# eddyxzc/lpopc

Measured on AMD Instinct MI355X. Metric: eval_g+eval_jac_g calls/sec, 4-phase 4096-LGR-pt problem, higher is better.
Workload: dtype f64

## Files before the change

lpopc_amd/csrc/problems/problems.hpp:

```cpp
#pragma once
#include <type_traits>
#include <hip/hip_runtime.h>

#include "../../../include/rpm_hip.h"

namespace rpm {

#define RPM_DEV __device__ __forceinline__

template <class P, class = void> struct prob_nq { static constexpr int value = 0; };
template <class P> struct prob_nq<P, decltype(void(P::NQ))> { static constexpr int value = P::NQ; };

template <class P, class CP>
RPM_DEV void pf_dae(int ph, double t, const double* x, const double* u, const double* p, CP c, double* f, double* cp) {
  if constexpr (prob_nq<P>::value > 0) P::dae(ph, t, x, u, p, c, f, cp);
  else P::dae(ph, t, x, u, c, f, cp);
}
template <class P, class = void>
struct has_stage : std::false_type {};
template <class P>
struct has_stage<P, std::void_t<typename P::Stage>> : std::true_type {};
template <class P, class = void>
struct stage_always : std::false_type {};
template <class P>
struct stage_always<P, std::enable_if_t<P::STAGE_ALWAYS>> : std::true_type {};
template <class P, bool = has_stage<P>::value>
struct stage_of { struct type {}; };
template <class P>
struct stage_of<P, true> { using type = typename P::Stage; };

template <class P, class CP>
RPM_DEV void pf_dae_jac_col(int ph, int v, double t, const double* x, const double* u, const double* p, CP c, double* df, double* dc) {
  if constexpr (prob_nq<P>::value > 0) P::dae_jac_col(ph, v, t, x, u, p, c, df, dc);
  else P::dae_jac_col(ph, v, t, x, u, c, df, dc);
}
template <class P>
RPM_DEV double pf_lagrange(int ph, double t, const double* x, const double* u, const double* p, const double* c) {
  if constexpr (prob_nq<P>::value > 0) return P::lagrange(ph, t, x, u, p, c);
  else return P::lagrange(ph, t, x, u, c);
}
template <class P>
RPM_DEV double pf_lagrange_grad_col(int ph, int v, double t, const double* x, const double* u, const double* p, const double* c) {
  if constexpr (prob_nq<P>::value > 0) return P::lagrange_grad_col(ph, v, t, x, u, p, c);
  else return P::lagrange_grad_col(ph, v, t, x, u, c);
}
template <class P>
RPM_DEV double pf_mayer(int ph, double t0, const double* x0, double tf, const double* xf, const double* p, const double* c) {
  if constexpr (prob_nq<P>::value > 0) return P::mayer(ph, t0, x0, tf, xf, p, c);
  else return P::mayer(ph, t0, x0, tf, xf, c);
}
template <class P>
RPM_DEV double pf_mayer_grad_col(int ph, int q, double t0, const double* x0, double tf, const double* xf, const double* p, const double* c) {
  if constexpr (prob_nq<P>::value > 0) return P::mayer_grad_col(ph, q, t0, x0, tf, xf, p, c);
  else return P::mayer_grad_col(ph, q, t0, x0, tf, xf, c);
}
template <class P>
RPM_DEV void pf_event(int ph, double t0, const double* x0, double tf, const double* xf, const double* p, const double* c, double* ev) {
  if constexpr (prob_nq<P>::value > 0) P::event(ph, t0, x0, tf, xf, p, c, ev);
  else P::event(ph, t0, x0, tf, xf, c, ev);
}
template <class P>
RPM_DEV void pf_event_jac_col(int ph, int v, double t0, const double* x0, double tf, const double* xf, const double* p, const double* c, double* de) {
  if constexpr (prob_nq<P>::value > 0) P::event_jac_col(ph, v, t0, x0, tf, xf, p, c, de);
  else P::event_jac_col(ph, v, t0, x0, tf, xf, c, de);
}
template <class P>
RPM_DEV void pf_link(int lph, int rph, const double* xl, const double* xr, const double* pl, const double* pr, const double* c, int nlink, double* lo) {
  if constexpr (prob_nq<P>::value > 0) P::link(lph, rph, xl, xr, pl, pr, c, nlink, lo);
  else P::link(lph, rph, xl, xr, c, nlink, lo);
}
template <class P>
RPM_DEV void pf_link_jac_col(int lph, int rph, int v, const double* xl, const double* xr, const double* pl, const double* pr, const double* c, int nlink, double* dl) {
  if constexpr (prob_nq<P>::value > 0) P::link_jac_col(lph, rph, v, xl, xr, pl, pr, c, nlink, dl);
  else P::link_jac_col(lph, rph, v, xl, xr, c, nlink, dl);
}

RPM_DEV double cube_rn(double x) {
  const double p = x * x, ep = fma(x, x, -p);
  const double q = p * x, eq = fma(p, x, -q);
  return q + (eq + ep * x);
}

struct LaunchProblem {
  static constexpr int ID = RPM_PROBLEM_LAUNCH;
  static constexpr int NX = 7, NU = 3, NC = 1, NE_MAX = 5, NLINK_MAX = 7, NCONST = 22;
  static constexpr bool HAS_ANALYTIC = false;

  template <class CP = const double*>
  RPM_DEV static void dae(int ph, double t, const double* x, const double* u, CP c,
                          double* f, double* p) {
    (void)t;
    const double r0 = x[0], r1 = x[1], r2 = x[2], m = x[6];
    const double rad = sqrt((r0 * r0 + r1 * r1) + r2 * r2);
    double vrel[3];
#pragma unroll
    for (int cc = 0; cc < 3; ++cc) {
      double ocr = 0.0;
      ocr += r0 * c[cc + 0];
      ocr += r1 * c[cc + 3];
      ocr += r2 * c[cc + 6];
      vrel[cc] = x[3 + cc] - ocr;
    }
    const double speedrel = sqrt((vrel[0] * vrel[0] + vrel[1] * vrel[1]) + vrel[2] * vrel[2]);
    const double altitude = rad - c[14];
    const double rho = exp(-altitude / c[13]) * c[12];
    const double bc = rho / (m * 2) * (c[11] * c[10]);
    const double bcspeed = bc * speedrel;
    const double mu3 = (1.0 * c[9]) / cube_rn(rad);
    double T_tot, mdot;
    if (ph == 1 || ph == 2) {
      const double T_srb = 1.0 * ((ph == 1 ? 6 : 3) * c[16]);
      const double T_first = 1.0 * c[17];
      T_tot = T_srb + T_first;
      double m1dot = 0.0, m2dot = 0.0;
      m1dot -= T_srb / (c[15] * c[19]);
      m2dot -= T_first / (c[15] * c[20]);
      mdot = m1dot + m2dot;
    } else if (ph == 3) {
      T_tot = 1.0 * c[17];
      mdot = 0.0;
      mdot -= T_tot / (c[15] * c[20]);
    } else {
      T_tot = 1.0 * c[18];
      mdot = 0.0;
      mdot -= T_tot / (c[15] * c[21]);
    }
    p[0] = (u[0] * u[0] + u[1] * u[1]) + u[2] * u[2];
    const double Toverm = T_tot / m;
#pragma unroll
    for (int j = 0; j < 3; ++j) {
      const double drag = (bcspeed * (-1.0)) * vrel[j];
      const double grav = (-mu3) * x[j];
      f[j] = x[3 + j];
      f[3 + j] = (Toverm * u[j] + drag) + grav;
    }
    f[6] = mdot;
  }

  struct Stage { double ocr[3], vrel[3], rho, mu3, speedrel, bc, T_tot, mdot; };
// ... 93 lines not shown
                            const double* c, double* ev) {
    (void)t0; (void)x0; (void)tf;
    if (ph != 4) return;
    const double mu = c[9];
    const double* rv = xf;
    const double* vv = xf + 3;
    double hv[3], nv[3], e3[3];
    hv[0] = rv[1] * vv[2] - rv[2] * vv[1];
    hv[1] = rv[2] * vv[0] - rv[0] * vv[2];
    hv[2] = rv[0] * vv[1] - rv[1] * vv[0];
    nv[0] = 0.0 * hv[2] - 1.0 * hv[1];
    nv[1] = 1.0 * hv[0] - 0.0 * hv[2];
    nv[2] = 0.0 * hv[1] - 0.0 * hv[0];
    const double n = sqrt(dot3(nv, nv));
    const double h2 = dot3(hv, hv);
    const double v2 = dot3(vv, vv);
    const double r = sqrt(dot3(rv, rv));
    const double s1 = v2 - mu / r, s2 = dot3(rv, vv);
#pragma unroll
    for (int j = 0; j < 3; ++j) e3[j] = (rv[j] * s1 - vv[j] * s2) * (1.0 / mu);
    const double p = h2 / mu;
    const double e = sqrt(dot3(e3, e3));
    const double twopi = 2 * 3.14159265358979323846;
    double Om1 = acos(nv[0] / n);
    if (nv[1] < 0 - 2.220446049250313e-16) Om1 = twopi - Om1;
    double Om2 = acos(dot3(nv, e3) / n / e);
    if (e3[2] < 0) Om2 = twopi - Om2;
    ev[0] = p / (1 - e * e);
    ev[1] = e;
    ev[2] = acos(hv[2] / sqrt(h2));
    ev[3] = Om1;
    ev[4] = Om2;
  }
  RPM_DEV static void link(int lph, int rph, const double* xfl, const double* x0r, const double* c,
                           int nlink, double* out) {
    (void)lph; (void)rph; (void)c;
    for (int j = 0; j < nlink; ++j) out[j] = x0r[j] - xfl[j];
  }
  RPM_DEV static double mayer(int ph, double t0, const double* x0, double tf, const double* xf,
                              const double* c) {
    (void)t0; (void)x0; (void)tf; (void)c;
    return ph == 4 ? -xf[6] : 0.0;
  }
  RPM_DEV static double lagrange(int ph, double t, const double* x, const double* u, const double* c) {
    (void)ph; (void)t; (void)x; (void)u; (void)c;
    return 0.0;
  }
};

struct HypersensitiveProblem {
  static constexpr int ID = RPM_PROBLEM_HYPERSENSITIVE;
  static constexpr int NX = 1, NU = 1, NC = 0, NE_MAX = 0, NLINK_MAX = 0, NCONST = 0;
  static constexpr bool HAS_ANALYTIC = true;
  template <class CP = const double*>
  RPM_DEV static void dae(int, double, const double* x, const double* u, CP, double* f, double*) {
    f[0] = ((-x[0]) * x[0]) * x[0] + u[0];
  }
  template <class CP = const double*>
  RPM_DEV static void dae_jac_col(int, int v, double, const double* x, const double*, CP,
                                  double* df, double*) {
    df[0] = (v == 0) ? -3 * (x[0] * x[0]) : (v == 1 ? 1.0 : 0.0);
  }
  RPM_DEV static void event(int, double, const double*, double, const double*, const double*, double*) {}
  RPM_DEV static void link(int, int, const double*, const double*, const double*, int, double*) {}
  RPM_DEV static double mayer(int, double, const double*, double, const double*, const double*) { return 0.0; }
  RPM_DEV static double lagrange(int, double, const double* x, const double* u, const double*) {
    return 0.5 * (x[0] * x[0] + u[0] * u[0]);
  }
  RPM_DEV static double lagrange_grad_col(int, int v, double, const double* x, const double* u, const double*) {
    return v == 0 ? x[0] : (v == 1 ? u[0] : 0.0);
  }
  RPM_DEV static double mayer_grad_col(int, int, double, const double*, double, const double*, const double*) {
    return 0.0;
  }
  RPM_DEV static void event_jac_col(int, int, double, const double*, double, const double*, const double*, double*) {}
  RPM_DEV static void link_jac_col(int, int, int, const double*, const double*, const double*, int, double*) {}
};

struct BrysonDenhamProblem {
  static constexpr int ID = RPM_PROBLEM_BRYSON_DENHAM;
  static constexpr int NX = 3, NU = 1, NC = 0, NE_MAX = 5, NLINK_MAX = 0, NCONST = 0;
  static constexpr bool HAS_ANALYTIC = false;
  template <class CP = const double*>
  RPM_DEV static void dae(int, double, const double* x, const double* u, CP, double* f, double*) {
    f[0] = x[1];
    f[1] = u[0];
    f[2] = 0.5 * (u[0] * u[0]);
  }
  RPM_DEV static void event(int, double, const double* x0, double, const double* xf, const double*, double* ev) {
    ev[0] = x0[0]; ev[1] = x0[1]; ev[2] = x0[2]; ev[3] = xf[0]; ev[4] = xf[1];
  }
  RPM_DEV static void link(int, int, const double*, const double*, const double*, int, double*) {}
  RPM_DEV static double mayer(int, double, const double*, double, const double* xf, const double*) { return xf[2]; }
  RPM_DEV static double lagrange(int, double, const double*, const double*, const double*) { return 0.0; }
};

struct BrachistochroneProblem {
  static constexpr int ID = RPM_PROBLEM_BRACHISTOCHRONE;
  static constexpr int NX = 3, NU = 1, NC = 0, NE_MAX = 5, NLINK_MAX = 0, NCONST = 1;
  static constexpr bool HAS_ANALYTIC = true;
  template <class CP = const double*>
  RPM_DEV static void dae(int, double, const double* x, const double* u, CP c, double* f, double*) {
    const double sn = sin(u[0]), cs = cos(u[0]);
    f[0] = x[2] * sn;
    f[1] = x[2] * cs;
    f[2] = c[0] * cs;
  }
  template <class CP = const double*>
  RPM_DEV static void dae_jac_col(int, int v, double, const double* x, const double* u, CP c,
                                  double* df, double*) {
    const double sn = sin(u[0]), cs = cos(u[0]);
    df[0] = df[1] = df[2] = 0.0;
    if (v == 2) { df[0] = sn; df[1] = cs; }
    if (v == 3) { df[0] = x[2] * cs; df[1] = -(x[2] * sn); df[2] = -(c[0] * sn); }
  }
  RPM_DEV static void event(int, double, const double* x0, double, const double* xf, const double*, double* ev) {
    ev[0] = x0[0]; ev[1] = x0[1]; ev[2] = x0[2]; ev[3] = xf[0]; ev[4] = xf[1];
  }
  RPM_DEV static void event_jac_col(int, int v, double, const double*, double, const double*, const double*, double* de) {
    for (int i = 0; i < 5; ++i) de[i] = 0.0;
    if (v < 3) de[v] = 1.0;
    if (v == 4) de[3] = 1.0;
    if (v == 5) de[4] = 1.0;
  }
  RPM_DEV static void link(int, int, const double*, const double*, const double*, int, double*) {}
  RPM_DEV static void link_jac_col(int, int, int, const double*, const double*, const double*, int, double*) {}
  RPM_DEV static double mayer(int, double, const double*, double tf, const double*, const double*) { return tf; }
  RPM_DEV static double mayer_grad_col(int, int v, double, const double*, double, const double*, const double*) {
    return v == 2 * NX + 1 ? 1.0 : 0.0;
  }
  RPM_DEV static double lagrange(int, double, const double*, const double*, const double*) { return 0.0; }
  RPM_DEV static double lagrange_grad_col(int, int, double, const double*, const double*, const double*) { return 0.0; }
};

struct MinTimeClimbProblem {
  static constexpr int ID = RPM_PROBLEM_MIN_TIME_CLIMB;
  static constexpr int NX = 4, NU = 1, NC = 0, NE_MAX = 7, NLINK_MAX = 0, NCONST = 10;
  static constexpr bool HAS_ANALYTIC = false;
  template <class CP = const double*>
  RPM_DEV static void dae(int, double, const double* x, const double* u, CP c, double* f, double*) {
    const double h = x[0], v = x[1], gam = x[2], m = x[3], al = u[0];
    const double r = h + c[0];
    const double rho = c[5] * exp(-h / c[6]);
    const double as = c[7] - c[8] * h;
    const double M = v / as;
    const double ch = cosh((M - 1.0) / 0.06);
    const double CLa = 3.44 + 1.0 / (ch * ch);
    const double CD0 = 0.013 + 0.0144 * (1.0 + tanh((M - 0.98) / 0.06));
    const double eta = 0.54 + 0.15 * (1.0 + tanh((M - 0.9) / 0.06));
    const double CD = CD0 + eta * CLa * (al * al);
    const double CL = CLa * al;
    const double q = 0.5 * rho * v * v;
    const double D = q * c[2] * CD;
    const double Lf = q * c[2] * CL;
    const double T = c[9] * pow(rho / c[5], 0.7) * (1.0 + 0.3 * M);
    const double sg = sin(gam), cg = cos(gam), sa = sin(al), ca = cos(al);
    f[0] = v * sg;
    f[1] = (T * ca - D) / m - c[1] * sg / (r * r);
    f[2] = (T * sa + Lf) / (m * v) + cg * (v / r - c[1] / (v * (r * r)));
    f[3] = -T / (c[3] * c[4]);
  }
  RPM_DEV static void event(int, double, const double* x0, double, const double* xf, const double*, double* ev) {
    ev[0] = x0[0]; ev[1] = x0[1]; ev[2] = x0[2]; ev[3] = x0[3]; ev[4] = xf[0]; ev[5] = xf[1]; ev[6] = xf[2];
  }
  RPM_DEV static void link(int, int, const double*, const double*, const double*, int, double*) {}
  RPM_DEV static double mayer(int, double, const double*, double tf, const double*, const double*) { return tf; }
  RPM_DEV static double lagrange(int, double, const double*, const double*, const double*) { return 0.0; }
};

struct QuadrotorProblem {
  static constexpr int ID = RPM_PROBLEM_QUADROTOR;
  static constexpr int NX = 12, NU = 4, NC = 0, NE_MAX = 0, NLINK_MAX = 0, NCONST = 15;
  static constexpr bool HAS_ANALYTIC = false;
  template <class CP = const double*>
  RPM_DEV static void dae(int, double, const double* x, const double* f4, CP c, double* f, double*) {
    const double ph = x[6], th = x[7], ps = x[8], p = x[9], q = x[10], r = x[11];
    const double F = ((f4[0] + f4[1]) + f4[2]) + f4[3];
    const double tx = c[2] * (f4[1] - f4[3]);
    const double ty = c[2] * (f4[2] - f4[0]);
    const double tz = c[6] * (((f4[0] - f4[1]) + f4[2]) - f4[3]);
    double sph, cph, sth, cth, sps, cps;
    sincos(ph, &sph, &cph);
    sincos(th, &sth, &cth);
    sincos(ps, &sps, &cps);
    const double b3x = cph * sth * cps + sph * sps;
    const double b3y = cph * sth * sps - sph * cps;
    const double b3z = cph * cth;
    const double Fm = F / c[0];
    f[0] = x[3];
    f[1] = x[4];
    f[2] = x[5];
    f[3] = Fm * b3x;
    f[4] = Fm * b3y;
    f[5] = Fm * b3z - c[1];
    const double w = q * sph + r * cph;
    f[6] = p + w * (sth / cth);
    f[7] = q * cph - r * sph;
    f[8] = w / cth;
    f[9] = (tx - (c[5] - c[4]) * q * r) / c[3];
    f[10] = (ty - (c[3] - c[5]) * p * r) / c[4];
    f[11] = (tz - (c[4] - c[3]) * p * q) / c[5];
  }
  struct Stage { double sph, cph, sth, cth, sps, cps; };
  static constexpr bool STAGE_ALWAYS = true;
  template <class CP = const double*>
  RPM_DEV static void stage(int, double, const double* x, const double*, CP, Stage& s) {
    sincos(x[6], &s.sph, &s.cph);
    sincos(x[7], &s.sth, &s.cth);
    sincos(x[8], &s.sps, &s.cps);
  }
  template <class CP = const double*>
  RPM_DEV static void dae_from(int, double, const double* x, const double* f4, CP c, const Stage& base, int var, double* f, double*) {
    Stage s = base;
    if (var == 6) sincos(x[6], &s.sph, &s.cph);
    else if (var == 7) sincos(x[7], &s.sth, &s.cth);
    else if (var == 8) sincos(x[8], &s.sps, &s.cps);
    const double p = x[9], q = x[10], r = x[11];
    const double F = ((f4[0] + f4[1]) + f4[2]) + f4[3];
    const double tx = c[2] * (f4[1] - f4[3]);
    const double ty = c[2] * (f4[2] - f4[0]);
    const double tz = c[6] * (((f4[0] - f4[1]) + f4[2]) - f4[3]);
    const double sph = s.sph, cph = s.cph, sth = s.sth, cth = s.cth, sps = s.sps, cps = s.cps;
    const double b3x = cph * sth * cps + sph * sps;
    const double b3y = cph * sth * sps - sph * cps;
    const double b3z = cph * cth;
    const double Fm = F / c[0];
    f[0] = x[3];
    f[1] = x[4];
    f[2] = x[5];
    f[3] = Fm * b3x;
    f[4] = Fm * b3y;
    f[5] = Fm * b3z - c[1];
    const double w = q * sph + r * cph;
    f[6] = p + w * (sth / cth);
    f[7] = q * cph - r * sph;
    f[8] = w / cth;
    f[9] = (tx - (c[5] - c[4]) * q * r) / c[3];
    f[10] = (ty - (c[3] - c[5]) * p * r) / c[4];
    f[11] = (tz - (c[4] - c[3]) * p * q) / c[5];
  }
  template <class CP = const double*>
  RPM_DEV static void dae_from2(int ph, double t, const double* x, const double* f4, CP c, const Stage& base, int va, int vb, double* f, double* p) {
    Stage s = base;
    if (va == 6 || vb == 6) sincos(x[6], &s.sph, &s.cph);
    if (va == 7 || vb == 7) sincos(x[7], &s.sth, &s.cth);
    if (va == 8 || vb == 8) sincos(x[8], &s.sps, &s.cps);
    dae_from(ph, t, x, f4, c, s, -1, f, p);
  }
  RPM_DEV static void event(int, double, const double*, double, const double*, const double*, double*) {}
  RPM_DEV static void link(int, int, const double*, const double*, const double*, int, double*) {}
  RPM_DEV static double mayer(int, double, const double*, double, const double*, const double*) { return 0.0; }
  RPM_DEV static double lagrange(int, double, const double* x, const double* f4, const double* c) {
    const double hov = c[0] * c[1] / 4.0;
    const double d0 = x[0] - c[7], d1 = x[1] - c[8], d2 = x[2] - c[9];
    const double ep = (d0 * d0 + d1 * d1) + d2 * d2;
    const double evv = (x[3] * x[3] + x[4] * x[4]) + x[5] * x[5];
    const double ea = (x[6] * x[6] + x[7] * x[7]) + x[8] * x[8];
    const double ew = (x[9] * x[9] + x[10] * x[10]) + x[11] * x[11];
    const double u0 = f4[0] - hov, u1 = f4[1] - hov, u2 = f4[2] - hov, u3 = f4[3] - hov;
    const double eu = ((u0 * u0 + u1 * u1) + u2 * u2) + u3 * u3;
    return (((c[10] * ep + c[11] * evv) + c[12] * ea) + c[13] * ew) + c[14] * eu;
  }
};

struct ParamSledProblem {
  static constexpr int ID = RPM_PROBLEM_PARAM_SLED;
  static constexpr int NX = 2, NU = 1, NQ = 1, NC = 0, NE_MAX = 4, NLINK_MAX = 0, NCONST = 1;
  static constexpr bool HAS_ANALYTIC = true;
  template <class CP = const double*>
  RPM_DEV static void dae(int, double, const double* x, const double* u, const double* p, CP, double* f, double*) {
    f[0] = x[1];
    f[1] = p[0] * u[0];
  }
  RPM_DEV static void event(int, double, const double* x0, double, const double* xf, const double*, const double*, double* ev) {
    ev[0] = x0[0];
    ev[1] = x0[1];
    ev[2] = xf[0];
    ev[3] = xf[1];
  }
  RPM_DEV static void link(int, int, const double*, const double*, const double*, const double*, const double*, int, double*) {}
  RPM_DEV static double mayer(int, double, const double*, double tf, const double*, const double* p, const double* c) {
    return tf + c[0] * (p[0] * p[0]);
  }
  RPM_DEV static double lagrange(int, double, const double*, const double*, const double*, const double*) { return 0.0; }
  template <class CP = const double*>
  RPM_DEV static void dae_jac_col(int, int v, double, const double*, const double* u, const double* p, CP, double* df, double*) {
    df[0] = (v == 1) ? 1.0 : 0.0;
    df[1] = (v == 2) ? p[0] : (v == 4 ? u[0] : 0.0);
  }
  RPM_DEV static void event_jac_col(int, int v, double, const double*, double, const double*, const double*, const double*, double* de) {
    de[0] = (v == 0) ? 1.0 : 0.0;
    de[1] = (v == 1) ? 1.0 : 0.0;
    de[2] = (v == 3) ? 1.0 : 0.0;
    de[3] = (v == 4) ? 1.0 : 0.0;
  }
  RPM_DEV static void link_jac_col(int, int, int, const double*, const double*, const double*, const double*, const double*, int, double*) {}
  RPM_DEV static double mayer_grad_col(int, int q, double, const double*, double, const double*, const double* p, const double* c) {
    return q == 5 ? 1.0 : (q == 6 ? 2.0 * c[0] * p[0] : 0.0);
  }
  RPM_DEV static double lagrange_grad_col(int, int, double, const double*, const double*, const double*, const double*) { return 0.0; }
};

struct ParamOscProblem {
  static constexpr int ID = RPM_PROBLEM_PARAM_OSC;
  static constexpr int NX = 2, NU = 1, NQ = 2, NC = 1, NE_MAX = 2, NLINK_MAX = 4, NCONST = 2;
  static constexpr bool HAS_ANALYTIC = false;
  template <class CP = const double*>
  RPM_DEV static void dae(int, double, const double* x, const double* u, const double* p, CP c, double* f, double* cp) {
    f[0] = x[1];
    f[1] = (-(p[0] * x[0]) - c[0] * x[1]) + u[0];
    cp[0] = x[0] + p[1] * u[0];
  }
  RPM_DEV static void event(int ph, double, const double* x0, double, const double* xf, const double* p, const double*, double* ev) {
    if (ph == 1) {
      ev[0] = x0[0];
      ev[1] = x0[1];
    } else {
      ev[0] = xf[0] + p[1];
    }
  }
  RPM_DEV static void link(int, int, const double* xl, const double* xr, const double* pl, const double* pr, const double*, int, double* lo) {
    lo[0] = xl[0] - xr[0];
    lo[1] = xl[1] - xr[1];
    lo[2] = pl[0] - pr[0];
    lo[3] = pl[1] - pr[1];
  }
  RPM_DEV static double mayer(int ph, double, const double*, double, const double* xf, const double* p, const double*) {
    return ph == 2 ? xf[0] * xf[0] + p[0] * p[1] : 0.0;
  }
  RPM_DEV static double lagrange(int, double, const double* x, const double* u, const double* p, const double* c) {
    return (u[0] * u[0] + p[1] * (x[0] * x[0])) + c[1] * (p[0] * p[0]);
  }
};

}
```

lpopc_amd/csrc/rpm_tile_kernels.hip:

```cpp
#include "rpm_device_internal.hpp"

namespace rpm {


template <class Prob, bool WG, bool WJ, bool AN, bool WAVE = false>
__device__ void endpoint_block(const KParams& K, const TaskDev task, const double* __restrict__ x,
                               double* __restrict__ g, double* __restrict__ vals, double* lds, int inst) {
  constexpr int NX = Prob::NX, NQ = prob_nq<Prob>::value, NQs = NQ > 0 ? NQ : 1;
  bool bad_g = false, bad_j = false;
  constexpr int NE = Prob::NE_MAX > 0 ? Prob::NE_MAX : 1;
  constexpr int NL = Prob::NLINK_MAX > 0 ? Prob::NLINK_MAX : 1;
  static_assert(!WAVE || 2 * NX + 3 + 2 * NQ <= 64, "endpoint perturbations must fit one wave");
  const int tid = WAVE ? int(threadIdx.x & 63) : int(threadIdx.x);
  const int nthr = WAVE ? 64 : int(blockDim.x);
  const double* c = K.consts + size_t(inst) * K.consts_stride;
  if (task.type == 0) {
    for (int r = tid; r < K.P + K.L; r += nthr) {
      if (WG) {
        double acc = 0.0;
        acc += K.alin_v[2 * r] * x[K.alin_j[2 * r]];
        acc += K.alin_v[2 * r + 1] * x[K.alin_j[2 * r + 1]];
        g[K.m_nl + r] = acc;
        chk_note(bad_g, acc);
      }
      if (WJ) {
        vals[K.nnz_nl + 2 * r] = K.alin_v[2 * r];
        vals[K.nnz_nl + 2 * r + 1] = K.alin_v[2 * r + 1];
      }
    }
  } else if (task.type == 1) {
    const PhaseDev ph = K.phases[task.idx];
    const int pi = tid;
    const bool act = pi <= 2 * NX + 2 + NQ;
    double x0[NX], xf[NX], ev[NE], pp[NQs];
#pragma unroll
    for (int j = 0; j < NQ; ++j) pp[j] = x[ph.x_t0 + 2 + j];
    double t0 = x[ph.x_t0], tf = x[ph.x_t0 + 1];
#pragma unroll
    for (int j = 0; j < NX; ++j) {
      x0[j] = x[ph.x_state0 + j * (ph.N + 1)];
      xf[j] = x[ph.x_state0 + j * (ph.N + 1) + ph.N];
    }
    double h = 1.0;
    if (WJ && !AN && pi >= 1) {
      const int v = pi - 1;
#pragma unroll
      for (int j = 0; j < NX; ++j) {
        if (v == j) { h = K.tol * (fabs(x0[j]) + 1); x0[j] += h; }
        if (v == NX + 1 + j) { h = K.tol * (fabs(xf[j]) + 1); xf[j] += h; }
      }
      if (v == NX) { h = K.tol * (1 + fabs(t0)); t0 += h; }
      if (v == 2 * NX + 1) { h = K.tol * (1 + fabs(tf)); tf += h; }
#pragma unroll
// ... 71 lines not shown
      }
    }
#pragma unroll
    for (int i = 0; i < NL; ++i) lo[i] = 0.0;
    if (act && (pi == 0 || !AN)) pf_link<Prob>(lk.left + 1, lk.right + 1, xl, xr, ql, qr, c, lk.nlink, lo);
    double base[NL];
    if constexpr (WAVE) {
#pragma unroll
      for (int i = 0; i < NL; ++i) base[i] = __shfl(lo[i], 0, 64);
    }
    if (pi == 0) {
#pragma unroll
      for (int i = 0; i < NL; ++i)
        if (i < lk.nlink) {
          if (!WAVE) lds[i] = lo[i];
          if (WG) { g[lk.g0 + i] = lo[i]; chk_note(bad_g, lo[i]); }
        }
    }
    if constexpr (!WAVE) {
      __syncthreads();
#pragma unroll
      for (int i = 0; i < NL; ++i) base[i] = lds[i];
    }
    if (WJ && act && pi >= 1) {
      const int v = pi - 1;
      double dl[NL];
      if constexpr (AN) {
        pf_link_jac_col<Prob>(lk.left + 1, lk.right + 1, v, xl, xr, ql, qr, c, lk.nlink, dl);
      } else {
#pragma unroll
        for (int i = 0; i < NL; ++i) dl[i] = (lo[i] - base[i]) / (1.0 * h);
      }
#pragma unroll
      for (int i = 0; i < NL; ++i)
        if (i < lk.nlink) { vals[lk.v0 + v * lk.nlink + i] = dl[i]; chk_note(bad_j, dl[i]); }
    }
  }
  chk_report(K.chk, bad_g, bad_j);
}


template <class Prob, bool WJ, bool AN, bool STG = false, class CP>
__device__ __forceinline__ void role_dynamics(int phase_num, int role, double tk, const double* xs, const double* us, CP c,
                                              double* f, double* cp,
                                              const typename stage_of<Prob>::type* base_stage = nullptr) {
  const int v = role - 1;
  if constexpr (STG) {
    Prob::dae_from(phase_num, tk, xs, us, c, *base_stage, (WJ && role >= 1) ? v : -1, f, cp);
  } else if (!AN || role == 0) {
    pf_dae<Prob>(phase_num, tk, xs, us, us + Prob::NU, c, f, cp);
  } else if constexpr (AN) {
    pf_dae_jac_col<Prob>(phase_num, v, tk, xs, us, us + Prob::NU, c, f, cp);
  }
}

template <int NX, int NU, int NQ>
__device__ __forceinline__ double perturb_uniform(int v, double pv, double tol, double* xs, double* us, double& tk) {
  const double h = tol * (1 + fabs(pv));
  const double pp = pv + h;
#pragma unroll
  for (int i = 0; i < NX; ++i) xs[i] = (v == i) ? pp : xs[i];
#pragma unroll
  for (int j = 0; j < NU; ++j) us[j] = (v == NX + j) ? pp : us[j];
  tk = (v == NX + NU) ? pp : tk;
#pragma unroll
  for (int j = 0; j < NQ; ++j) us[NU + j] = (v == NX + NU + 1 + j) ? pp : us[NU + j];
  return h;
}

template <class Prob, int T, bool WG, bool CHK>
__device__ __forceinline__ void publish_base(const double* f, const double* cp, double* Fb, int kk, double* g, int g0, int N,
                                             int k, bool& bad_g) {
  constexpr int NX = Prob::NX, NC = Prob::NC;
#pragma unroll
  for (int i = 0; i < NX; ++i) Fb[i * T + kk] = f[i];
#pragma unroll
  for (int j = 0; j < NC; ++j) {
    Fb[(NX + j) * T + kk] = cp[j];
    if (WG) {
      g[g0 + (NX + j) * N + k] = cp[j];
      if (CHK) chk_note(bad_g, cp[j]);
    }
  }
}

template <int T, bool CHK>
__device__ __forceinline__ void store_defect(int sv, double dx, double tspan, const double* Fb, int kk, double* g, int g0,
                                             int N, int k, bool& bad_g) {
  const double dfc = dx - Fb[sv * T + kk] * (tspan / 2.0);
  g[g0 + sv * N + k] = dfc;
  if (CHK) chk_note(bad_g, dfc);
}

__device__ __forceinline__ int xcd_place(int b, int count) {
  const int per = count >> 3, rem = count & 7, xcd = b & 7;
  return xcd * per + (xcd < rem ? xcd : rem) + (b >> 3);
}

#define RPM_REC(rec, f) __builtin_amdgcn_readfirstlane((rec)[offsetof(TileDev, f) / 4])

template <class Prob, int T, bool WG, bool WJ, bool AN, bool DXM = false>
__global__ void rpm_tile_kernel(const KParams K, const double* __restrict__ xall,
                                double* __restrict__ gall, double* __restrict__ vall) {
  constexpr int NX = Prob::NX, NU = Prob::NU, NC = Prob::NC, NQ = prob_nq<Prob>::value;
  constexpr int NO = NX + NC;
  constexpr int NV = NX + NU + 1 + NQ;
// ... 60 lines not shown
  const int sv = WJ ? role - 1 : role;
  double dx = 0.0;
  if (WG && !DXM && sv >= 0 && sv < NX) {
    const double* drow = Ds + (nd.drow_off - tl.drow0);
    const double* xcol = Xs + sv * K.max_span + (nd.dcol0 - tl.span0);
    for (int j = 0; j < nd.dlen; ++j) dx += drow[j] * xcol[j];
  }
  if constexpr (DXM && WG) {
    if (tid < 64) {
      typedef double d4 __attribute__((ext_vector_type(4)));
      const int lr = tid & 15, kq = tid >> 4;
      const int ksteps = (tl.span_len + 3) >> 2;
      for (int rb = 0; rb < T; rb += 16) {
        const int row = rb + lr;
        const bool row_ok = row < tl.cnt;
        const NodeDev ndr = K.nodes[ph.node0 + tl.k0 + (row_ok ? row : tl.cnt - 1)];
        const int rel0 = ndr.dcol0 - tl.span0;
        const double* drow = Ds + (ndr.drow_off - tl.drow0);
        for (int cb = 0; cb < NX; cb += 16) {
          const int st = cb + lr;
          d4 acc = {0.0, 0.0, 0.0, 0.0};
          for (int s = 0; s < ksteps; ++s) {
            const int kcol = 4 * s + kq;
            const int rel = kcol - rel0;
            const double a = (row_ok && rel >= 0 && rel < ndr.dlen) ? drow[rel] : 0.0;
            const double b = (st < NX && kcol < tl.span_len) ? Xs[st * K.max_span + kcol] : 0.0;
            acc = __builtin_amdgcn_mfma_f64_16x16x4f64(a, b, acc, 0, 0, 0);
          }
#pragma unroll
          for (int i = 0; i < 4; ++i) {
            const int orow = rb + kq + 4 * i;
            if (st < NX && orow < tl.cnt) DXs[st * T + orow] = acc[i];
          }
        }
      }
    }
  }

  double h = 1.0;
  const int v = role - 1;
  if (WJ && !AN && role >= 1) {
#pragma unroll
    for (int i = 0; i < NX; ++i)
      if (v == i) { h = K.tol * (1 + fabs(xs[i])); xs[i] += h; }
#pragma unroll
    for (int j = 0; j < NU; ++j)
      if (v == NX + j) { h = K.tol * (1 + fabs(us[j])); us[j] += h; }
    if (v == NX + NU) { h = K.tol * (1 + fabs(tk)); tk += h; }
#pragma unroll
    for (int j = 0; j < NQ; ++j)
      if (v == NX + NU + 1 + j) { h = K.tol * (1 + fabs(us[NU + j])); us[NU + j] += h; }
  }
  double f[NX > 0 ? NX : 1], cp[NCs];
  role_dynamics<Prob, WJ, AN>(ph.phase_num, role, tk, xs, us, c, f, cp);
  if (role == 0 && act) publish_base<Prob, T, WG, true>(f, cp, Fb, kk, g, ph.g0, ph.N, k, bad_g);
  __syncthreads();

  if (act) {
    const int N = ph.N;
    if (WG && sv >= 0 && sv < NX) store_defect<T, true>(sv, DXM ? DXs[sv * T + kk] : dx, tspan, Fb, kk, g, ph.g0, N, k, bad_g);
    if (WJ && role >= 1) {
      double J[NO];
#pragma unroll
      for (int o = 0; o < NO; ++o) {
        const double pert = o < NX ? f[o < NX ? o : 0] : cp[o >= NX ? o - NX : 0];
        J[o] = AN ? pert : (pert - Fb[o * T + kk]) / h;
      }
      double* vb = vals + ph.v_nl0 + k;
      if (v != NX + NU) {
        const int bv = v < NX + NU ? v : v + 1;
#pragma unroll
        for (int o = 0; o < NO; ++o) {
          double val;
          if (o < NX) {
            const double ret = J[o] * (tf - t0) / 2.0;
            val = (o == v) ? ddiag - ret : -ret;
          } else {
            val = J[o];
          }
          vb[size_t(o * NB + bv) * N] = val;
          chk_note(bad_j, val);
        }
      } else {
        const double a0 = -(tau * 0.5) + 0.5, af = (tau * 0.5) + 0.5;
#pragma unroll
        for (int o = 0; o < NO; ++o) {
          double v0, vf;
          if (o < NX) {
            const double fb = Fb[o * T + kk];
            const double dt = J[o] * (tf - t0) / 2.0;
            v0 = fb * (0.5) - a0 * dt;
            vf = -fb * (0.5) + af * dt;
          } else {
            v0 = a0 * J[o];
            vf = af * J[o];
          }
          vb[size_t(o * NB + NX + NU) * N] = v0;
          vb[size_t(o * NB + NX + NU + 1) * N] = vf;
          chk_note(bad_j, v0);
          chk_note(bad_j, vf);
        }
      }
    }
  }
  chk_report(K.chk, bad_g, bad_j);

  if (WJ && !K.skip_const) {
    const double* __restrict__ src = K.doff_vals + tl.c_src0;
    double* __restrict__ dst = vals + tl.c_dst0;
#pragma unroll
    for (int u = 0; u < CPRE; ++u) {
      const int q = tid + u * nthr;
      if (q < tl.c_cnt) {
#pragma unroll
        for (int i = 0; i < NX; ++i) dst[size_t(i) * tl.c_stride + q] = cpre[u];
      }
    }
    for (int q = tid + CPRE * nthr; q < tl.c_cnt; q += nthr) {
      const double dv = src[q];
// ... 38 lines not shown
  const int k = tl.k0 + kc;
  const int nidx = ph.node0 + k;
  const double tau = K.points[nidx];
  const NodeDev nd = K.nodes[nidx];
  const double ddiag = WJ ? K.diag[nidx] : 0.0;
  for (int q = tid; q < NX * tl.span_len; q += NTHR) {
    const int i = q / tl.span_len, r = q - i * tl.span_len;
    Xs[i * K.max_span + r] = x[ph.x_state0 + i * (ph.N + 1) + tl.span0 + r];
  }
  for (int q = tid; q < NU * tl.cnt; q += NTHR) {
    const int j = q / tl.cnt, r = q - j * tl.cnt;
    Us[j * T + r] = x[ph.x_control0 + j * ph.N + tl.k0 + r];
  }
  if (WG)
    for (int q = tid; q < tl.drow_len; q += NTHR) Ds[q] = K.dvals[tl.drow0 + q];
  const double t0 = x[ph.x_t0], tf = x[ph.x_t0 + 1];
  RPM_TRC(1);
  __syncthreads();
  RPM_TRC(2);

  const bool node_ok = kk < tl.cnt;
  const double tspan = tf - t0;
  const double tk0 = (tau + 1) * (tspan / 2.0) + t0;
  const int N = ph.N;
  bool first = true, no_chk = false;
  for (int role = grp; role < R || first; role += RG) {
    const bool act = node_ok && role < R;
    double xs[NX > 0 ? NX : 1], us[NU + NQ > 0 ? NU + NQ : 1];
#pragma unroll
    for (int i = 0; i < NX; ++i) xs[i] = Xs[i * K.max_span + (k - tl.span0)];
#pragma unroll
    for (int j = 0; j < NU; ++j) us[j] = Us[j * T + kc];
#pragma unroll
    for (int j = 0; j < NQ; ++j) us[NU + j] = x[ph.x_t0 + 2 + j];
    double tk = tk0;
    const int sv = WJ ? role - 1 : role;
    double dx = 0.0;
    if (WG && sv >= 0 && sv < NX) {
      const double* drow = Ds + (nd.drow_off - tl.drow0);
      const double* xcol = Xs + sv * K.max_span + (nd.dcol0 - tl.span0);
      for (int j = 0; j < nd.dlen; ++j) dx += drow[j] * xcol[j];
    }
    double h = 1.0;
    const int v = role - 1;
    if (WJ && !AN && role >= 1) {
      double pv;
      if (v < NX) pv = Xs[v * K.max_span + (k - tl.span0)];
      else if (v < NX + NU) pv = Us[(v - NX) * T + kc];
      else if (v == NX + NU) pv = tk;
      else pv = x[ph.x_t0 + 1 + (v - NX - NU)];
      h = perturb_uniform<NX, NU, NQ>(v, pv, K.tol, xs, us, tk);
    }
    double f[NX > 0 ? NX : 1], cp[NCs];
    role_dynamics<Prob, WJ, AN>(ph.phase_num, role, tk, xs, us, c, f, cp);
    if (first) {
      if (role == 0 && act) publish_base<Prob, T, WG, false>(f, cp, Fb, kk, g, ph.g0, N, k, no_chk);
      __syncthreads();
      RPM_TRC(3);
      first = false;
    }
    if (act) {
      if (WG && sv >= 0 && sv < NX) store_defect<T, false>(sv, dx, tspan, Fb, kk, g, ph.g0, N, k, no_chk);
      if (WJ && role >= 1) {
        double J[NO];
#pragma unroll
        for (int o = 0; o < NO; ++o) {
          const double pert = o < NX ? f[o < NX ? o : 0] : cp[o >= NX ? o - NX : 0];
          J[o] = AN ? pert : (pert - Fb[o * T + kk]) / h;
        }
        double* vb = vals + ph.v_nl0 + k;
        if (v != NX + NU) {
          const int bv = v < NX + NU ? v : v + 1;
#pragma unroll
          for (int o = 0; o < NO; ++o) {
            double val;
            if (o < NX) {
              const double ret = J[o] * (tf - t0) / 2.0;
              val = (o == v) ? ddiag - ret : -ret;
            } else {
              val = J[o];
            }
            vb[size_t(o * NB + bv) * N] = val;
          }
        } else {
          const double a0 = -(tau * 0.5) + 0.5, af = (tau * 0.5) + 0.5;
#pragma unroll
          for (int o = 0; o < NO; ++o) {
            double v0, vf;
            if (o < NX) {
              const double fb = Fb[o * T + kk];
              const double dt = J[o] * (tf - t0) / 2.0;
              v0 = fb * (0.5) - a0 * dt;
              vf = -fb * (0.5) + af * dt;
            } else {
              v0 = a0 * J[o];
              vf = af * J[o];
            }
            vb[size_t(o * NB + NX + NU) * N] = v0;
            vb[size_t(o * NB + NX + NU + 1) * N] = vf;
          }
        }
      }
    }
  }
  RPM_TRC(4);
  if (WJ && !K.skip_const) {
    const double* __restrict__ src = K.doff_vals + tl.c_src0;
    double* __restrict__ dst = vals + tl.c_dst0;
    const int lead = int((reinterpret_cast<size_t>(dst) >> 3) & 15);
    for (int q = tid - lead; q < tl.c_cnt; q += NTHR) {
      if (q >= 0) {
        const double dv = src[q];
#pragma unroll
        for (int i = 0; i < NX; ++i) dst[size_t(i) * tl.c_stride + q] = dv;
      }
    }
  }
#ifdef RPM_DIAG
  RPM_TRC(5);
  if (K.trace) {
    __builtin_amdgcn_s_waitcnt(0);
// ... 293 lines not shown
      for (int j = 0; j < NU; ++j) us0[j] = Us[j * T + kc];
      const double tau0 = cur[S_TAU + kc], t00 = cur[S_TT], tf0 = cur[S_TT + 1];
      Prob::stage(phase_num, (tau0 + 1) * ((tf0 - t00) / 2.0) + t00, xs0, us0, c4, base_stage);
    }
    for (int role = grp; role < R || first; role += RG) {
      const bool act = node_ok && role < R;
#ifdef RPM_DIAG
      const bool trc = role == 5;
      if (trc) { RPM_PTRC(jt, 24); }
#endif
      double xs[NXs], us[NUs];
#pragma unroll
      for (int i = 0; i < NX; ++i) xs[i] = Xs[i * K.max_span + (k - span0)];
#pragma unroll
      for (int j = 0; j < NU; ++j) us[j] = Us[j * T + kc];
#pragma unroll
      for (int j = 0; j < NQ; ++j) us[NU + j] = cur[S_TT + 2 + j];
      double tk;
      {
        const double tau = cur[S_TAU + kc], t0 = cur[S_TT], tf = cur[S_TT + 1];
        tk = (tau + 1) * ((tf - t0) / 2.0) + t0;
      }
      const int sv = WJ ? role - 1 : role;
      double dx = 0.0;
      if (WG && !DXM && sv >= 0 && sv < NX) {
        const NodeDev nd = reinterpret_cast<const NodeDev*>(cur + S_ND)[kc];
        const double* drow = Ds + (nd.drow_off - drow0);
        const double* xcol = Xs + sv * K.max_span + (nd.dcol0 - span0);
        int j = 0;
        for (; j + 4 <= nd.dlen; j += 4) {
          const double d0 = drow[j], d1 = drow[j + 1], d2 = drow[j + 2], d3 = drow[j + 3];
          const double x0 = xcol[j], x1 = xcol[j + 1], x2 = xcol[j + 2], x3 = xcol[j + 3];
          dx += d0 * x0;
          dx += d1 * x1;
          dx += d2 * x2;
          dx += d3 * x3;
        }
        for (; j < nd.dlen; ++j) dx += drow[j] * xcol[j];
      }
#ifdef RPM_DIAG
      if (trc) { if (dx == 1e300) xs[0] = 0; RPM_PTRC(jt, 25); }
#endif
      double h = 1.0;
      const int v = role - 1;
      if (WJ && !AN && role >= 1) {
        double pv;
        if (v < NX) pv = Xs[v * K.max_span + (k - span0)];
        else if (v < NX + NU) pv = Us[(v - NX) * T + kc];
        else if (v == NX + NU) pv = tk;
        else pv = cur[S_TT + 1 + (v - NX - NU)];
        h = perturb_uniform<NX, NU, NQ>(v, pv, K.tol, xs, us, tk);
      }
      double f[NXs], cp[NCs];
      role_dynamics<Prob, WJ, AN, STG>(phase_num, role, tk, xs, us, c4, f, cp, &base_stage);
#ifdef RPM_DIAG
      if (trc) { if (f[0] == 1e300) cp[0] = 0; RPM_PTRC(jt, 26); }
#endif
      if (first) {
        if (role == 0 && act) publish_base<Prob, T, WG, false>(f, cp, Fb, kk, g, g0, N, k, no_chk);
        if (grp < 4) { RPM_PTRC(jt, grp * 4 + 1); }
        if (grp == 0) {
          __hip_atomic_store(fb_ready, jt + 1, __ATOMIC_RELEASE, __HIP_MEMORY_SCOPE_WORKGROUP);
        } else {
          while (__hip_atomic_load(fb_ready, __ATOMIC_ACQUIRE, __HIP_MEMORY_SCOPE_WORKGROUP) < jt + 1)
            __builtin_amdgcn_s_sleep(1);
        }
        if (grp < 4) { RPM_PTRC(jt, grp * 4 + 2); }
        first = false;
      }
      if (act) {
        const double tau = cur[S_TAU + kc], t0 = cur[S_TT], tf = cur[S_TT + 1];
        const double ddiag = cur[S_DG + kc];
        if (WG && sv >= 0 && sv < NX) {
          if constexpr (DXM) {
            while (__hip_atomic_load(dx_ready, __ATOMIC_ACQUIRE, __HIP_MEMORY_SCOPE_WORKGROUP) < NDMA * (jt + 1)) __builtin_amdgcn_s_sleep(1);
            dx = DXs[sv * T + kk];
          }
          store_defect<T, false>(sv, dx, tf - t0, Fb, kk, g, g0, N, k, no_chk);
        }
        if (WJ && role >= 1) {
          double J[NO];
#pragma unroll
          for (int o = 0; o < NO; ++o) {
            const double pert = o < NX ? f[o < NX ? o : 0] : cp[o >= NX ? o - NX : 0];
            J[o] = AN ? pert : (pert - Fb[o * T + kk]) / h;
          }
          double* __restrict__ vb = vals + v_nl0;
          if (v != NX + NU) {
            const int bv = v < NX + NU ? v : v + 1;
#pragma unroll
            for (int o = 0; o < NO; ++o) {
              double val;
              if (o < NX) {
                const double ret = J[o] * (tf - t0) / 2.0;
                val = (o == v) ? ddiag - ret : -ret;
              } else {
                val = J[o];
              }
              (vb + size_t(o * NB + bv) * N)[k] = val;
            }
          } else {
            const double a0 = -(tau * 0.5) + 0.5, af = (tau * 0.5) + 0.5;
#pragma unroll
            for (int o = 0; o < NO; ++o) {
              double v0, vf;
              if (o < NX) {
                const double fb = Fb[o * T + kk];
                const double dt = J[o] * (tf - t0) / 2.0;
                v0 = fb * (0.5) - a0 * dt;
                vf = -fb * (0.5) + af * dt;
              } else {
                v0 = a0 * J[o];
                vf = af * J[o];
              }
              (vb + size_t(o * NB + NX + NU) * N)[k] = v0;
              (vb + size_t(o * NB + NX + NU + 1) * N)[k] = vf;
            }
          }
        }
      }
#ifdef RPM_DIAG
      if (trc) { RPM_PTRC(jt, 27); }
#endif
    }
    if (grp < 4) { RPM_PTRC(jt, grp * 4 + 3); }
    if (jt == n_iter - 1) { RPM_PEDGE_MAX(23); }
  }
}

static size_t pl_lds_bytes(int nx, int nu, int nc, int nq, const KParams& kp, bool dxm) {
  const PlLds L(nx, nu, nc, nq, kp.max_span, kp.max_drow, kp.max_cshare, true, dxm);
  return size_t(pl_shape(nx + nu + 2 + nq).NH) * L.half * sizeof(double);
}

void tile_pipeline_setup(Engine& e, Device* d, const ProblemDims& pd, int device_id) {
    int ncu = 0;
    if (hipDeviceGetAttribute(&ncu, hipDeviceAttributeMultiprocessorCount, device_id) != hipSuccess || ncu <= 0) ncu = 256;
    const int max_c = d->kp.max_cshare;
// ... 153 lines not shown
```

Before: 651,300.

## Skip time-perturbation dynamics for autonomous problems and use reciprocal FD division

Adds an AUTONOMOUS trait to every problem. For those problems the finite-difference role that perturbs time (role 1+NX+NU) reuses the base dynamics from shared memory instead of re-evaluating the DAE, since f does not depend on t. It also replaces the per-output division by h with one reciprocal plus an FMA-corrected quotient, and falls back to true division when operands are outside a safe exponent range. This removes one dynamics evaluation per column and several f64 divides, at the cost of extra branching and range checks.

Result: no change. 653,100 (median of 4 runs) (+0.3%).

```diff
diff --git a/lpopc_amd/csrc/problems/problems.hpp b/lpopc_amd/csrc/problems/problems.hpp
--- a/lpopc_amd/csrc/problems/problems.hpp
+++ b/lpopc_amd/csrc/problems/problems.hpp
@@ -21,6 +21,10 @@
 template <class P>
 struct has_stage<P, std::void_t<typename P::Stage>> : std::true_type {};
 template <class P, class = void>
+struct prob_autonomous : std::false_type {};
+template <class P>
+struct prob_autonomous<P, std::enable_if_t<P::AUTONOMOUS>> : std::true_type {};
+template <class P, class = void>
 struct stage_always : std::false_type {};
 template <class P>
 struct stage_always<P, std::enable_if_t<P::STAGE_ALWAYS>> : std::true_type {};
@@ -85,6 +89,7 @@
   static constexpr int ID = RPM_PROBLEM_LAUNCH;
   static constexpr int NX = 7, NU = 3, NC = 1, NE_MAX = 5, NLINK_MAX = 7, NCONST = 22;
   static constexpr bool HAS_ANALYTIC = false;
+  static constexpr bool AUTONOMOUS = true;
 
   template <class CP = const double*>
   RPM_DEV static void dae(int ph, double t, const double* x, const double* u, CP c,
@@ -284,6 +289,7 @@
   static constexpr int ID = RPM_PROBLEM_HYPERSENSITIVE;
   static constexpr int NX = 1, NU = 1, NC = 0, NE_MAX = 0, NLINK_MAX = 0, NCONST = 0;
   static constexpr bool HAS_ANALYTIC = true;
+  static constexpr bool AUTONOMOUS = true;
   template <class CP = const double*>
   RPM_DEV static void dae(int, double, const double* x, const double* u, CP, double* f, double*) {
     f[0] = ((-x[0]) * x[0]) * x[0] + u[0];
@@ -313,6 +319,7 @@
   static constexpr int ID = RPM_PROBLEM_BRYSON_DENHAM;
   static constexpr int NX = 3, NU = 1, NC = 0, NE_MAX = 5, NLINK_MAX = 0, NCONST = 0;
   static constexpr bool HAS_ANALYTIC = false;
+  static constexpr bool AUTONOMOUS = true;
   template <class CP = const double*>
   RPM_DEV static void dae(int, double, const double* x, const double* u, CP, double* f, double*) {
     f[0] = x[1];
@@ -331,6 +338,7 @@
   static constexpr int ID = RPM_PROBLEM_BRACHISTOCHRONE;
   static constexpr int NX = 3, NU = 1, NC = 0, NE_MAX = 5, NLINK_MAX = 0, NCONST = 1;
   static constexpr bool HAS_ANALYTIC = true;
+  static constexpr bool AUTONOMOUS = true;
   template <class CP = const double*>
   RPM_DEV static void dae(int, double, const double* x, const double* u, CP c, double* f, double*) {
     const double sn = sin(u[0]), cs = cos(u[0]);
@@ -369,6 +377,7 @@
   static constexpr int ID = RPM_PROBLEM_MIN_TIME_CLIMB;
   static constexpr int NX = 4, NU = 1, NC = 0, NE_MAX = 7, NLINK_MAX = 0, NCONST = 10;
   static constexpr bool HAS_ANALYTIC = false;
+  static constexpr bool AUTONOMOUS = true;
   template <class CP = const double*>
   RPM_DEV static void dae(int, double, const double* x, const double* u, CP c, double* f, double*) {
     const double h = x[0], v = x[1], gam = x[2], m = x[3], al = u[0];
@@ -404,6 +413,7 @@
   static constexpr int ID = RPM_PROBLEM_QUADROTOR;
   static constexpr int NX = 12, NU = 4, NC = 0, NE_MAX = 0, NLINK_MAX = 0, NCONST = 15;
   static constexpr bool HAS_ANALYTIC = false;
+  static constexpr bool AUTONOMOUS = true;
   template <class CP = const double*>
   RPM_DEV static void dae(int, double, const double* x, const double* f4, CP c, double* f, double*) {
     const double ph = x[6], th = x[7], ps = x[8], p = x[9], q = x[10], r = x[11];
@@ -499,6 +509,7 @@
   static constexpr int ID = RPM_PROBLEM_PARAM_SLED;
   static constexpr int NX = 2, NU = 1, NQ = 1, NC = 0, NE_MAX = 4, NLINK_MAX = 0, NCONST = 1;
   static constexpr bool HAS_ANALYTIC = true;
+  static constexpr bool AUTONOMOUS = true;
   template <class CP = const double*>
   RPM_DEV static void dae(int, double, const double* x, const double* u, const double* p, CP, double* f, double*) {
     f[0] = x[1];
@@ -537,6 +548,7 @@
   static constexpr int ID = RPM_PROBLEM_PARAM_OSC;
   static constexpr int NX = 2, NU = 1, NQ = 2, NC = 1, NE_MAX = 2, NLINK_MAX = 4, NCONST = 2;
   static constexpr bool HAS_ANALYTIC = false;
+  static constexpr bool AUTONOMOUS = true;
   template <class CP = const double*>
   RPM_DEV static void dae(int, double, const double* x, const double* u, const double* p, CP c, double* f, double* cp) {
     f[0] = x[1];
diff --git a/lpopc_amd/csrc/rpm_fd_div.hpp b/lpopc_amd/csrc/rpm_fd_div.hpp
--- /dev/null
+++ b/lpopc_amd/csrc/rpm_fd_div.hpp
@@ -0,0 +1,58 @@
+#pragma once
+
+#if defined(__HIP__) || defined(__CUDACC__)
+#define RPM_FD_HD __host__ __device__ inline __attribute__((always_inline))
+#else
+#define RPM_FD_HD inline
+#endif
+
+namespace rpm {
+
+constexpr double FD_SAFE_LO = 0x1p-500, FD_SAFE_HI = 0x1p+500;
+
+struct FdRecip { double h, r; bool ok; };
+
+RPM_FD_HD FdRecip fd_recip(double h) {
+  const double ah = __builtin_fabs(h);
+  return FdRecip{h, 1.0 / h, ah >= FD_SAFE_LO && ah <= FD_SAFE_HI};
+}
+
+RPM_FD_HD double fd_quot_step(const FdRecip& rc, double a, bool& safe) {
+  const double q0 = a * rc.r;
+  const double e = __builtin_fma(-rc.h, q0, a);
+  const double aa = __builtin_fabs(a);
+  unsigned long long bits;
+  __builtin_memcpy(&bits, &a, sizeof bits);
+  safe = bool(int(safe) & ((int(aa >= FD_SAFE_LO) & int(aa <= FD_SAFE_HI)) | int(bits == 0)));
+  return __builtin_fma(e, rc.r, q0);
+}
+
+RPM_FD_HD double fd_quot(const FdRecip& rc, double a) {
+  bool safe = rc.ok;
+  const double q = fd_quot_step(rc, a, safe);
+  return safe ? q : a / rc.h;
+}
+
+template <int N, class Num>
+RPM_FD_HD void fd_quot_column(const FdRecip& rc, Num num, double* q) {
+  constexpr int G = 4;
+#if defined(__clang__)
+#pragma unroll
+#endif
+  for (int o0 = 0; o0 < N; o0 += G) {
+    double a[G];
+    bool safe = rc.ok;
+#if defined(__clang__)
+#pragma unroll
+#endif
+    for (int o = o0; o < (o0 + G < N ? o0 + G : N); ++o) q[o] = fd_quot_step(rc, a[o - o0] = num(o), safe);
+    if (!safe) {
+#if defined(__clang__)
+#pragma unroll
+#endif
+      for (int o = o0; o < (o0 + G < N ? o0 + G : N); ++o) q[o] = a[o - o0] / rc.h;
+    }
+  }
+}
+
+}
diff --git a/lpopc_amd/csrc/rpm_tile_kernels.hip b/lpopc_amd/csrc/rpm_tile_kernels.hip
--- a/lpopc_amd/csrc/rpm_tile_kernels.hip
+++ b/lpopc_amd/csrc/rpm_tile_kernels.hip
@@ -1,4 +1,5 @@
 #include "rpm_device_internal.hpp"
+#include "rpm_fd_div.hpp"
 
 namespace rpm {
 
@@ -176,6 +177,18 @@
   } else if constexpr (AN) {
     pf_dae_jac_col<Prob>(phase_num, v, tk, xs, us, us + Prob::NU, c, f, cp);
   }
+}
+
+template <class Prob, bool WJ, bool AN>
+__device__ __forceinline__ bool role_repeats_base(int role) {
+  return prob_autonomous<Prob>::value && WJ && !AN && role == 1 + Prob::NX + Prob::NU;
+}
+template <class Prob, int T>
+__device__ __forceinline__ void fetch_base(const double* Fb, int kk, double* f, double* cp) {
+#pragma unroll
+  for (int i = 0; i < Prob::NX; ++i) f[i] = Fb[i * T + kk];
+#pragma unroll
+  for (int j = 0; j < Prob::NC; ++j) cp[j] = Fb[(Prob::NX + j) * T + kk];
 }
 
 template <int NX, int NU, int NQ>
@@ -342,19 +355,23 @@
       if (v == NX + NU + 1 + j) { h = K.tol * (1 + fabs(us[NU + j])); us[NU + j] += h; }
   }
   double f[NX > 0 ? NX : 1], cp[NCs];
-  role_dynamics<Prob, WJ, AN>(ph.phase_num, role, tk, xs, us, c, f, cp);
+  const bool repeats = role_repeats_base<Prob, WJ, AN>(role);
+  if (!repeats) role_dynamics<Prob, WJ, AN>(ph.phase_num, role, tk, xs, us, c, f, cp);
   if (role == 0 && act) publish_base<Prob, T, WG, true>(f, cp, Fb, kk, g, ph.g0, ph.N, k, bad_g);
   __syncthreads();
+  if (repeats) fetch_base<Prob, T>(Fb, kk, f, cp);
 
   if (act) {
     const int N = ph.N;
     if (WG && sv >= 0 && sv < NX) store_defect<T, true>(sv, DXM ? DXs[sv * T + kk] : dx, tspan, Fb, kk, g, ph.g0, N, k, bad_g);
     if (WJ && role >= 1) {
       double J[NO];
-#pragma unroll
-      for (int o = 0; o < NO; ++o) {
-        const double pert = o < NX ? f[o < NX ? o : 0] : cp[o >= NX ? o - NX : 0];
-        J[o] = AN ? pert : (pert - Fb[o * T + kk]) / h;
+      const auto pert = [&](int o) { return o < NX ? f[o < NX ? o : 0] : cp[o >= NX ? o - NX : 0]; };
+      if constexpr (AN) {
+#pragma unroll
+        for (int o = 0; o < NO; ++o) J[o] = pert(o);
+      } else {
+        fd_quot_column<NO>(fd_recip(h), [&](int o) { return pert(o) - Fb[o * T + kk]; }, J);
       }
       double* vb = vals + ph.v_nl0 + k;
       if (v != NX + NU) {
@@ -499,7 +516,8 @@
       h = perturb_uniform<NX, NU, NQ>(v, pv, K.tol, xs, us, tk);
     }
     double f[NX > 0 ? NX : 1], cp[NCs];
-    role_dynamics<Prob, WJ, AN>(ph.phase_num, role, tk, xs, us, c, f, cp);
+    if (role_repeats_base<Prob, WJ, AN>(role) && !first) fetch_base<Prob, T>(Fb, kk, f, cp);
+    else role_dynamics<Prob, WJ, AN>(ph.phase_num, role, tk, xs, us, c, f, cp);
     if (first) {
       if (role == 0 && act) publish_base<Prob, T, WG, false>(f, cp, Fb, kk, g, ph.g0, N, k, no_chk);
       __syncthreads();
@@ -510,10 +528,12 @@
       if (WG && sv >= 0 && sv < NX) store_defect<T, false>(sv, dx, tspan, Fb, kk, g, ph.g0, N, k, no_chk);
       if (WJ && role >= 1) {
         double J[NO];
-#pragma unroll
-        for (int o = 0; o < NO; ++o) {
-          const double pert = o < NX ? f[o < NX ? o : 0] : cp[o >= NX ? o - NX : 0];
-          J[o] = AN ? pert : (pert - Fb[o * T + kk]) / h;
+        const auto pert = [&](int o) { return o < NX ? f[o < NX ? o : 0] : cp[o >= NX ? o - NX : 0]; };
+        if constexpr (AN) {
+#pragma unroll
+          for (int o = 0; o < NO; ++o) J[o] = pert(o);
+        } else {
+          fd_quot_column<NO>(fd_recip(h), [&](int o) { return pert(o) - Fb[o * T + kk]; }, J);
         }
         double* vb = vals + ph.v_nl0 + k;
         if (v != NX + NU) {
@@ -913,7 +933,8 @@
         h = perturb_uniform<NX, NU, NQ>(v, pv, K.tol, xs, us, tk);
       }
       double f[NXs], cp[NCs];
-      role_dynamics<Prob, WJ, AN, STG>(phase_num, role, tk, xs, us, c4, f, cp, &base_stage);
+      if (role_repeats_base<Prob, WJ, AN>(role) && !first) fetch_base<Prob, T>(Fb, kk, f, cp);
+      else role_dynamics<Prob, WJ, AN, STG>(phase_num, role, tk, xs, us, c4, f, cp, &base_stage);
 #ifdef RPM_DIAG
       if (trc) { if (f[0] == 1e300) cp[0] = 0; RPM_PTRC(jt, 26); }
 #endif
@@ -941,10 +962,12 @@
         }
         if (WJ && role >= 1) {
           double J[NO];
-#pragma unroll
-          for (int o = 0; o < NO; ++o) {
-            const double pert = o < NX ? f[o < NX ? o : 0] : cp[o >= NX ? o - NX : 0];
-            J[o] = AN ? pert : (pert - Fb[o * T + kk]) / h;
+          const auto pert = [&](int o) { return o < NX ? f[o < NX ? o : 0] : cp[o >= NX ? o - NX : 0]; };
+          if constexpr (AN) {
+#pragma unroll
+            for (int o = 0; o < NO; ++o) J[o] = pert(o);
+          } else {
+            fd_quot_column<NO>(fd_recip(h), [&](int o) { return pert(o) - Fb[o * T + kk]; }, J);
           }
           double* __restrict__ vb = vals + v_nl0;
           if (v != NX + NU) {
```
